# scalar-labs/jepsen

Hardware: AMD Instinct MI355X
Metric: history ops verified/sec (node), independent cas-register 10k keys, 1/2/4/8 GPU (higher is better)
Workload: dtype int64

## Files before the change

jepsen_amd/csrc/jh_lin.hip:

```cpp
#include "jh_internal.h"
#include <hipcub/hipcub.hpp>
#include <algorithm>
#include <type_traits>
#include "lin/lin_common.h"

namespace {

constexpr int F_READ = 0, F_WRITE = 1, F_CAS = 2, F_OTHER = 4;
constexpr int T_INVOKE = 0, T_OK = 1, T_FAIL = 2, T_INFO = 3;
constexpr uint64_t VIOL_NONE = ~0ULL;
#ifndef JH_LDS_TBL
#define JH_LDS_TBL 0
#endif
constexpr int LDS_TBL = JH_LDS_TBL;
#ifdef JH_STEP_PROF
#define PROF_MARK(v) const unsigned long long v = __builtin_amdgcn_s_memtime()
#define PROF_ADD(acc, a, b) acc += (b) - (a)
#else
#define PROF_MARK(v)
#define PROF_ADD(acc, a, b)
#endif
#ifdef JH_DFS_STATS
#define DFS_STAT(x) x
#else
#define DFS_STAT(x)
#endif
template <int LG_BKT, int LG_BLOOM>
struct MemoCfg {
    static constexpr int LG = LG_BKT;
    static constexpr int BKT = 1 << LG_BKT;
    static constexpr int SLOTS = BKT * 4;
    static constexpr int EVICT = SLOTS * 5 / 8;
    static constexpr int BLOOM = 1 << LG_BLOOM;
    static constexpr int OFF_MEMO = LDS_TBL;
    static constexpr int OFF_BLOOM = OFF_MEMO + SLOTS * 8;
    static constexpr int OFF_CNT = OFF_BLOOM + BLOOM / 8;
    static constexpr int LDS = OFF_CNT + BKT;
};
#ifndef JH_MEMOQ_LG
#define JH_MEMOQ_LG 7
#define JH_MEMOQ_BLOOM 14
#endif
using MemoQ = MemoCfg<JH_MEMOQ_LG, JH_MEMOQ_BLOOM>;
#ifndef JH_MEMOH_BLOOM
#define JH_MEMOH_BLOOM 17
#endif
using MemoH = MemoCfg<12, JH_MEMOH_BLOOM>;
using MemoM = MemoCfg<10, 15>;
#ifndef JH_P2_LG
#define JH_P2_LG 10
#define JH_P2_BLOOM 17
#endif
#ifndef JH_P2_PER_CU
#define JH_P2_PER_CU 3
#endif
using MemoP2 = MemoCfg<JH_P2_LG, JH_P2_BLOOM>;
constexpr int P2_DENSE_PER_CU = 6;
using MemoP2D = MemoCfg<9, 16>;
constexpr int P2_LEAN_PER_CU = P2_DENSE_PER_CU;
constexpr int STATE_BITS = 20, T_BITS = 20, GEN_BITS = 24;
constexpr uint32_t STATE_MASK = (1u << STATE_BITS) - 1, T_MASK = (1u << T_BITS) - 1;

struct Rec {
    int32_t proc;
    uint8_t type, f;
    uint16_t pad;
    int32_t v1, v2;
};

struct Op {
    int32_t v1, v2;
    int32_t rr;
    int32_t fa;
// ... 641 lines not shown
#endif
__device__ __forceinline__ uint32_t hbm_insert(uint64_t *memo, uint32_t cap_mask, uint32_t gen,
                                               uint32_t ct, uint32_t cs, uint64_t cm) {
    uint32_t b = (uint32_t)memo_hash(ct, cs, cm) & cap_mask & ~(HB - 1);
    const uint64_t w1 = ((uint64_t)gen << 40) | ((uint64_t)ct << 20) | cs;
    for (;;) {
        const ulonglong2 *B = (const ulonglong2 *)(memo + 2 * (size_t)b);
        ulonglong2 e[HB];
#pragma unroll
        for (uint32_t j = 0; j < HB; j++) e[j] = B[j];
        int j0 = -1;
        unsigned long long exp = 0;
#pragma unroll
        for (int j = HB - 1; j >= 0; j--)
            if ((e[j].y >> 40) != gen) { j0 = j; exp = e[j].y; }
        if (j0 < 0) { b = (b + HB) & cap_mask; continue; }
        if (__hip_atomic_compare_exchange_strong((unsigned long long *)&memo[2 * (size_t)(b + j0) + 1],
                                                 &exp, (unsigned long long)w1,
                                                 __ATOMIC_RELAXED, __ATOMIC_RELAXED,
                                                 __HIP_MEMORY_SCOPE_WORKGROUP)) {
            __hip_atomic_store(&memo[2 * (size_t)(b + j0)], cm, __ATOMIC_RELAXED,
                               __HIP_MEMORY_SCOPE_WORKGROUP);
#ifdef JH_DUP_WRITE
            if (g_dup_base)
                g_dup_base[((uintptr_t)&memo[2 * (size_t)(b + j0)] >> 4) & ((1u << 26) - 1)] = make_ulonglong2(cm, w1);
#endif
            return b + (uint32_t)j0;
        }
    }
}

__device__ __forceinline__ uint64_t hbm_probe(const uint64_t *memo, uint32_t cap_mask, uint32_t gen,
                                              uint32_t ct, uint32_t cs, uint64_t cm,
                                              unsigned long long &probes) {
    const uint64_t w1want = ((uint64_t)gen << 40) | ((uint64_t)ct << 20) | cs;
    uint32_t b = (uint32_t)memo_hash(ct, cs, cm) & cap_mask & ~(HB - 1);
    for (;;) {
        const ulonglong2 *B = (const ulonglong2 *)(memo + 2 * (size_t)b);
        ulonglong2 e[HB];
#pragma unroll
        for (uint32_t j = 0; j < HB; j++) e[j] = B[j];
        probes++;
        int empty = -1, hit = -1;
#pragma unroll
        for (int j = HB - 1; j >= 0; j--) {
            if ((e[j].y >> 40) != gen) empty = j;
            if (e[j].y == w1want && e[j].x == cm) hit = j;
        }
        if (hit >= 0 && (empty < 0 || hit < empty)) return b + (uint32_t)hit;
        if (empty >= 0) return (1ULL << 32) | (b + (uint32_t)empty);
        b = (b + HB) & cap_mask;
    }
}

__device__ __forceinline__ uint32_t lk_t(uint64_t k) { return (uint32_t)(k >> 48) & 0x3FFF; }
__device__ __forceinline__ uint32_t lk_s(uint64_t k) { return (uint32_t)(k >> 40) & 0xFF; }
__device__ __forceinline__ uint64_t lk_m(uint64_t k) { return k & ((1ULL << 40) - 1); }
__device__ __forceinline__ void lk_hash(uint32_t klo, uint32_t khi, uint32_t &h1, uint32_t &h2) {
    h1 = (klo ^ __builtin_rotateleft32(khi, 16)) * 0x9E3779B1u;
    h2 = (klo + __builtin_rotateleft32(khi, 5)) * 0x85EBCA77u;
}
template <class M>
__device__ __forceinline__ void lk_bkts(uint32_t h1, uint32_t h2, uint32_t &b1, uint32_t &b2) {
    b1 = h1 >> (32 - M::LG);
    b2 = h2 >> (32 - M::LG);
}
__device__ __forceinline__ uint32_t lk_bl(uint32_t h) { return h ^ (h >> 15); }

template <class M>
__device__ __noinline__ uint64_t memo_evict(uint64_t *lmemo, uint32_t *bcnt, uint32_t *bloom,
                                            uint64_t *memo, uint64_t *stage,
                                            uint32_t cap_mask, uint32_t gen, uint32_t t_cur,
                                            uint32_t theta_old, int lane,
                                            uint32_t *hlog = nullptr, uint32_t hlog_cap = 0, uint32_t nlog = 0) {
    static_assert(M::SLOTS < 65536, "kept fits 16 bits");
    int bins = 0;
#pragma unroll 1
    for (int r = 0; r < M::SLOTS / 64; r++) {
        const uint64_t x = lmemo[lane + 64 * r];
        stage[lane + 64 * r] = x;
        const uint32_t xt = lk_t(x);
        const int d = x == 0 ? 99 : (xt >= t_cur ? 0 : (int)min(t_cur - xt, 15u));
#pragma unroll
        for (int b = 0; b < 16; b++) {
            const int cnt = __popcll(ballot(d == b));
            if (lane == b) bins += cnt;
        }
    }
    int acc = 0, dstar = -1;
#pragma unroll 1
    for (int b = 0; b < 16; b++) {
        acc += readlane(bins, b);
        if (acc > M::EVICT / 2) break;
        dstar = b;
    }
    uint32_t th2;
    if (dstar < 0) th2 = t_cur + 1;
    else {
        th2 = t_cur > (uint32_t)dstar ? t_cur - (uint32_t)dstar : 0u;
        if (dstar == 15) th2 = t_cur - min(t_cur, 15u);
    }
    th2 = max(th2, theta_old);
    wave_sync();
#pragma unroll 1
    for (int r = 0; r < M::SLOTS / 64; r++) lmemo[lane + 64 * r] = 0;
    for (int i = lane; i < M::BKT / 4; i += 64) bcnt[i] = 0;
// ... 330 lines not shown
                    const uint32_t x = (uint32_t)readlane((int)drq, (int)(u - 1 - tb0));
                    if (lane == ru) wrq = x;
                    w++;
                }
                t = pt;
                r = lay_hi(t) & 63;
                DFS_STAT(n_reload++);
            }
            PROF_MARK(q5); PROF_ADD(pc_pop, q2, q5);
        }
        if (depth >= A.stack_cap) { verdict = JH_UNKNOWN; if (lane == 0) atomicOr(A.flags, QF_STACK_OVERFLOW); break; }
    }
    inserts = ins;
    tmax_out = tmax;
#ifdef JH_STEP_PROF
    if (A.dbg && lane == 0) {
        unsigned long long *d = A.dbg + 16 * (size_t)blockIdx.x;
        d[10] += pc_lift; d[11] += pc_probe; d[12] += pc_ins; d[13] += pc_fwd; d[14] += pc_pop;
        d[0] += pc_cand; d[1] += pc_key; d[8] += pc_lds;
    }
#endif
#ifdef JH_DFS_STATS
    if (A.dbg && lane == 0) {
        unsigned long long *d = A.dbg + 16 * (size_t)blockIdx.x;
        d[4] += n_steps; d[5] += (unsigned long long)ins; d[6] += n_evict; d[7] += n_reload; d[9] += n_slow;
    }
#endif
    return verdict;
}

template <class M, bool HO = false>
__device__ __forceinline__ int dfs_lean(const DfsArgs &A, const KeyInfo &K, const char *tb, int key, int lane,
                        uint64_t *memo, Frame *stack, uint64_t *stage,
                        long long &inserts, uint32_t &tmax_out, unsigned long long &my_probes,
                        uint32_t &ins_real, uint32_t *hlog) {
    const OpC *ops = (const OpC *)tb;
    const Lay *lay = (const Lay *)(tb + tblc_ops_bytes(K));
    const uint32_t n_ok = (uint32_t)K.n_ok;
    const int n_ops = K.n_ops;
    const uint32_t cap_mask = A.memo_cap - 1;
    const uint32_t gen = (A.gen_base + (uint32_t)key + 1) & ((1u << GEN_BITS) - 1);
    uint64_t *lmemo = (uint64_t *)(jh_lds + M::OFF_MEMO);
    uint32_t *bloom = (uint32_t *)(jh_lds + M::OFF_BLOOM);
    uint32_t *bcnt = (uint32_t *)(jh_lds + M::OFF_CNT);
    uint8_t *bcnt8 = (uint8_t *)bcnt;
    for (int i = lane; i < M::SLOTS; i += 64) lmemo[i] = 0;
    for (int i = lane; i < M::BKT / 4; i += 64) bcnt[i] = 0;
    for (int i = lane; i < M::BLOOM / 32; i += 64) bloom[i] = 0;
    const uint32_t lb_lo = lane < 32 ? 1u << lane : 0u, lb_hi = lane >= 32 ? 1u << (lane - 32) : 0u;
    uint32_t theta = 0;
    int lcount = 0;
    uint32_t n_steps = 0, n_lay = 0, n_up = 0, n_spill = 0, n_refill = 0, n_slow = 0, n_evict = 0, n_hbm = 0;
    const unsigned long long probes0 = my_probes;

    uint32_t tb0 = 0, drq = 0, dhi = 0;
    auto load_lay = [&](uint32_t base) {
        DFS_STAT(n_lay++);
        tb0 = base;
        const uint32_t u = base + (uint32_t)lane;
        if (u < n_ok) { const Lay e = lay[u]; drq = e.rq; dhi = e.hi; }
    };
    auto lay_hi = [&](uint32_t u) -> uint32_t {
        if (u - tb0 >= 64u) load_lay(u >= 32 ? u - 32 : 0);
        return (uint32_t)readlane((int)dhi, (int)(u - tb0));
    };
    int pb = 0;
    uint32_t urq = RQ_EMPTY;
    auto load_up = [&](int base) {
        DFS_STAT(n_up++);
        pb = base;
        const int j = base + lane;
        urq = j < n_ops ? ops[j].rq : RQ_EMPTY;
    };
    uint32_t fm_lo = 0, fm_hi = 0, f_ti = 0, f_s = 0, fr_lo = 0, fr_hi = 0;

    load_lay(0);
    uint32_t t = 0, tmax = 0, depth = 0, ring_lo = 0;
    uint64_t mask = 0;
    uint32_t s = (uint32_t)A.init_state;
    int verdict = -1;
    uint32_t ins = 0;
    uint32_t budget = (uint32_t)min<int64_t>(A.budget, 0x7FFFFFFF);
    uint32_t chk = min(budget, 1023u);
    int w = (int)(lay_hi(0) >> 6), P = w;
    uint32_t r = lay_hi(0) & 63;
    uint32_t rn = n_ok > 1 ? (lay_hi(1) & 63) : 0;
    uint32_t wrq = lane < w ? ops[lane].rq : RQ_EMPTY;
    load_up(P);
    wave_sync();
    uint32_t ins_saved = 0xFFFFFFFFu;
    uint32_t nlog = 0;
    uint32_t stall_base = 0, stall_tmax = 0;
    bool ho = false;
    unsigned long long ho_off = 0;
    auto advance = [&](uint32_t nt) {
        for (uint32_t u = t; u < nt; u++) {
            const uint32_t ru = u == t ? r : (lay_hi(u) & 63);
            const uint32_t sh = (uint32_t)wave_shl1((int)wrq);
            if (lane >= (int)ru) wrq = sh;
            w--;
            if (lane == w) wrq = RQ_EMPTY;
            const int c = (int)(lay_hi(u + 1) >> 6);
            if (c > 0) {
                if (P < pb || P + c > pb + 64) load_up(c <= 32 && P >= 32 ? P - 32 : P);
                for (int kk = 0; kk < c; kk++) {
                    const uint32_t x = (uint32_t)readlane((int)urq, P - pb + kk);
                    if (lane == w + kk) wrq = x;
                }
                w += c; P += c;
            }
        }
    };
    if (A.rs_mode == 2 && A.rs_off) {
        const int64_t ro = A.rs_off[key];
        if (ro >= 0) {
            const uint64_t *hd = (const uint64_t *)(A.rs_arena + ro);
            const uint64_t h_mask = hd[0], h_ts = hd[1], h_dt = hd[2], h_ins = hd[3], h_n = hd[4];
            const uint32_t d = (uint32_t)h_dt;
            if (d <= A.stack_cap && h_n <= (uint64_t)A.memo_cap / 4) {
                const Frame *fsrc = (const Frame *)(hd + 8);
                const ulonglong2 *ent = (const ulonglong2 *)(fsrc + d);
                uint32_t tmx = 0;
                for (uint32_t j = (uint32_t)lane; j < (uint32_t)h_n; j += 64) {
                    const ulonglong2 e = ent[j];
                    const uint32_t et = (uint32_t)(e.y >> 20) & T_MASK, es = (uint32_t)e.y & STATE_MASK;
                    const uint32_t sl = hbm_insert(memo, cap_mask, gen, et, es, e.x);
                    if constexpr (HO) { if (hlog && j < A.hlog_cap) hlog[j] = sl; } else (void)sl;
                    uint32_t g1, g2;
                    lk_hash((uint32_t)e.x, (uint32_t)(e.x >> 32) | (et << 16) | (es << 8) | 0x80000000u, g1, g2);
                    bloom_set2<M>(bloom, lk_bl(g1), lk_bl(g2));
                    tmx = max(tmx, et + 1);
                }
                for (int o = 32; o > 0; o >>= 1) tmx = max(tmx, (uint32_t)__shfl_xor((int)tmx, o));
                theta = rflu(tmx);
                if constexpr (HO) nlog = (uint32_t)min<uint64_t>(h_n, 0xFFFFu);
                ring_lo = d > 32 ? d - 32 : 0;
                for (uint32_t j = (uint32_t)lane; j < ring_lo; j += 64) stack[j] = fsrc[j];
                {
                    const uint32_t idx = ring_lo + (((uint32_t)lane - ring_lo) & 63);
                    if (idx < d) {
                        const Frame fr = fsrc[idx];
                        fm_lo = (uint32_t)fr.mask; fm_hi = (uint32_t)(fr.mask >> 32); f_ti = fr.t_i;
                        f_s = (uint32_t)fr.s; fr_lo = (uint32_t)fr.rest; fr_hi = (uint32_t)(fr.rest >> 32);
                    }
                }
                __builtin_amdgcn_fence(__ATOMIC_RELEASE, "workgroup");
                __builtin_amdgcn_fence(__ATOMIC_ACQUIRE, "workgroup");
                wave_sync();
                depth = d;
                mask = h_mask;
                s = (uint32_t)(h_ts >> 32);
                ins = (uint32_t)h_ins;
                chk = min(budget, ins);
                const uint32_t nt = (uint32_t)h_ts;
                advance(nt);
                t = nt;
                tmax = max((uint32_t)(h_dt >> 32), t);
                r = lay_hi(t) & 63;
                rn = t + 1 < n_ok ? (lay_hi(t + 1) & 63) : 0;
                stall_base = ins; stall_tmax = tmax;
            }
        }
    }
    const ulonglong2 *B = (const ulonglong2 *)lmemo;
    uint64_t absent = 0, nm_r = 0;
    uint32_t u_r = 0, klo = 0, khi = 0, b1 = 0, b2 = 0, n1 = 0, n2 = 0, h1 = 0, h2 = 0, nvl = 0;
    auto child_keys = [&]() {
        u_r = t; nm_r = 0;
        if ((absent >> r) & 1) {
            uint64_t nm = drop_bit(mask, r);
            uint32_t u = t + 1;
            if (u >= n_ok) nm = 0;
            else if ((nm >> rn) & 1) {
                uint32_t ru = rn;
                for (;;) {
                    nm = drop_bit(nm, ru);
                    u++;
                    if (u >= n_ok) { nm = 0; break; }
                    ru = lay_hi(u) & 63;
                    if (!((nm >> ru) & 1)) break;
                }
            }
            u_r = u; nm_r = nm;
        }
        nvl = wrq >> 16;
        const bool is_r = lane == (int)r;
        const uint32_t hi_a = (uint32_t)(mask >> 32) | (t << 16) | 0x80000000u;
        const uint32_t hi_r = (uint32_t)(nm_r >> 32) | (u_r << 16) | 0x80000000u;
        klo = is_r ? (uint32_t)nm_r : ((uint32_t)mask | lb_lo);
        khi = (is_r ? hi_r : (hi_a | lb_hi)) | (nvl << 8);
        lk_hash(klo, khi, h1, h2);
        lk_bkts<M>(h1, h2, b1, b2);
    };

expand:
    DFS_STAT(n_steps++);
    {
        const uint32_t req = wrq & 0xFFFF;
        absent = (ballot(req == s) | ballot(req == RQ_ANY)) & ~mask;
    }
    if (!absent) goto pop;
    child_keys();
    {
        const bool cl = (absent >> lane) & 1;
        const uint32_t a1 = cl ? b1 : 0u, a2 = cl ? b2 : 0u;
        const uint64_t k = ((uint64_t)khi << 32) | klo;
        n1 = bcnt8[a1]; n2 = bcnt8[a2];
        __builtin_amdgcn_sched_barrier(0);
        const ulonglong2 x0 = B[2 * a1], x1 = B[2 * a1 + 1];
        const ulonglong2 y0 = B[2 * a2], y1 = B[2 * a2 + 1];
        const uint64_t hit = ballot(x0.x == k) | ballot(x0.y == k) | ballot(x1.x == k) | ballot(x1.y == k) |
                             ballot(y0.x == k) | ballot(y0.y == k) | ballot(y1.x == k) | ballot(y1.y == k);
        absent &= ~hit;
        if (t < theta && absent) {
            DFS_STAT(n_slow++);
            uint64_t low = absent;
            if (u_r >= theta) low &= ~(1ULL << r);
            const uint32_t kt = khi >> 16 & 0x7FFF, ks = (khi >> 8) & 0xFF;
            const uint64_t km = k & ((1ULL << 40) - 1);
            const bool maybe = ((low >> lane) & 1) && bloom_test2<M>(bloom, lk_bl(h1), lk_bl(h2));
            bool found = false;
            if (maybe) found = (hbm_probe(memo, cap_mask, gen, kt, ks, km, my_probes) >> 32) == 0;
            absent &= ~ballot(found);
        }
    }
    if (!absent) goto pop;

insert:
    {
        if (ins >= chk) {
            if (ins >= budget && !extend_budget(A, budget)) { verdict = JH_UNKNOWN; goto done; }
            if (handover(A, ins)) { ins_saved = ins; ins = budget; verdict = JH_UNKNOWN; goto done; }
            if (A.claim) {
                int c = 0;
                if (lane == 0) c = __hip_atomic_load(&A.claim[key], __ATOMIC_RELAXED, __HIP_MEMORY_SCOPE_AGENT);
                if (readlane(c, 0)) { verdict = JH_CANCELLED; goto done; }
            }
            if (A.prio_ins > 0 && ins >= (uint32_t)A.prio_ins) {
                if (ins >= 4u * (uint32_t)A.prio_ins) __builtin_amdgcn_s_setprio(3);
                else if (ins >= 2u * (uint32_t)A.prio_ins) __builtin_amdgcn_s_setprio(2);
                else __builtin_amdgcn_s_setprio(1);
            }
            if (!std::is_same<M, MemoQ>::value && A.stall) {
                if (tmax > stall_tmax) { stall_tmax = tmax; stall_base = ins; }
                if (lane == 0)
                    __hip_atomic_store(&A.stall[key], ins - stall_base, __ATOMIC_RELAXED, __HIP_MEMORY_SCOPE_AGENT);
            }
            if (HO && A.handoff) {
                int h = 0;
                if (lane == 0) h = __hip_atomic_load(&A.handoff[key], __ATOMIC_RELAXED, __HIP_MEMORY_SCOPE_AGENT);
                if (readlane(h, 0) == HO_ASK) {
                    bool ok = hlog && nlog <= A.hlog_cap && ins <= A.memo_cap / 4;
                    if (ok) {
                        const uint64_t bytes = 64 + (uint64_t)depth * sizeof(Frame) + (uint64_t)ins * 16;
                        unsigned long long off = 0;
                        if (lane == 0) off = atomicAdd(A.rs_used, (unsigned long long)((bytes + 255) & ~255ULL));
                        ho_off = readlane64(off, 0);
                        ok = ho_off + bytes <= A.rs_cap;
                    }
                    int won = 0;
                    if (lane == 0) {
                        int exp = HO_ASK;
                        won = __hip_atomic_compare_exchange_strong(&A.handoff[key], &exp, ok ? HO_SAVING : HO_REFUSED,
                                                                   __ATOMIC_RELAXED, __ATOMIC_RELAXED,
                                                                   __HIP_MEMORY_SCOPE_AGENT) ? 1 : 0;
                    }
                    if (readlane(won, 0) && ok) { ho = true; goto done; }
                }
            }
            chk = min(budget, ins + (HO && A.handoff ? 256u : 1024u));
        }
        const int i = __builtin_ctzll(absent);
        ins++;
        const uint32_t ns = (uint32_t)readlane((int)nvl, i);
        const bool to_r = (uint32_t)i == r;
        const uint32_t nt = to_r ? u_r : t;
        {
            const bool pick1 = n1 <= n2;
            const uint32_t bs = pick1 ? b1 : b2, nsl = pick1 ? n1 : n2;
            const uint64_t full_m = ballot(nsl >= 4);
            if (!((full_m >> i) & 1)) {
                if (lane == i) {
                    lmemo[4 * bs + nsl] = ((uint64_t)khi << 32) | klo;
                    bcnt8[bs] = (uint8_t)(nsl + 1);
                }
                if (++lcount >= M::EVICT) {
                    DFS_STAT(n_evict++);
                    const uint64_t er = memo_evict<M>(lmemo, bcnt, bloom, memo, stage, cap_mask, gen, nt, theta, lane,
                                                      hlog, A.hlog_cap, nlog);
                    DFS_STAT(n_hbm += (uint32_t)lcount - ((uint32_t)er & 0xFFFF));
                    lcount = rfl((int)((uint32_t)er & 0xFFFF));
                    nlog = rflu(((uint32_t)er >> 16) & 0xFFFF);
                    theta = rflu((uint32_t)(er >> 32));
                }
            } else {
                const uint64_t nmask = to_r ? nm_r : (mask | (1ULL << i));
                if (lane == i) {
                    const uint32_t sl = hbm_insert(memo, cap_mask, gen, nt, ns, nmask);
                    bloom_set2<M>(bloom, lk_bl(h1), lk_bl(h2));
                    if (hlog && nlog < A.hlog_cap) hlog[nlog] = sl;
                }
                nlog = min(nlog + 1, 0xFFFFu);
                __builtin_amdgcn_fence(__ATOMIC_RELEASE, "workgroup");
                __builtin_amdgcn_fence(__ATOMIC_ACQUIRE, "workgroup");
                theta = max(theta, nt + 1);
                DFS_STAT(n_hbm++);
            }
        }
        if (depth - ring_lo == 64) {
            DFS_STAT(n_spill++);
            const uint32_t kk = ((uint32_t)lane - ring_lo) & 63;
            if (kk < 32) {
                Frame fr;
                fr.mask = ((uint64_t)fm_hi << 32) | fm_lo; fr.t_i = f_ti; fr.s = (int32_t)f_s;
                fr.rest = ((uint64_t)fr_hi << 32) | fr_lo; fr.pad[0] = fr.pad[1] = 0;
                stack[ring_lo + kk] = fr;
            }
            ring_lo += 32;
        }
        {
            const uint64_t nrest = absent & (absent - 1);
            const bool me = lane == (int)(depth & 63);
            fm_lo = me ? (uint32_t)mask : fm_lo;
            fm_hi = me ? (uint32_t)(mask >> 32) : fm_hi;
            f_ti = me ? ((t << 6) | (uint32_t)i) : f_ti;
            f_s = me ? s : f_s;
            fr_lo = me ? (uint32_t)nrest : fr_lo;
            fr_hi = me ? (uint32_t)(nrest >> 32) : fr_hi;
        }
        depth++;
        s = ns;
        if (!to_r) {
            mask |= 1ULL << i;
            goto expand;
        }
        mask = nm_r;
        if (nt >= n_ok) { t = nt; tmax = max(tmax, t); verdict = JH_VALID; goto done; }
        advance(nt);
        t = nt;
        if (t > tmax) {
            tmax = t;
            if (A.stamp_progress && A.seq_start && lane == 0)
                __hip_atomic_store(&A.seq_start[key], __builtin_amdgcn_s_memrealtime() | 1ULL, __ATOMIC_RELAXED,
                                   __HIP_MEMORY_SCOPE_AGENT);
        }
        r = lay_hi(t) & 63;
        rn = t + 1 < n_ok ? (lay_hi(t + 1) & 63) : 0;
        goto expand;
    }

pop:
    DFS_STAT(n_steps++);
    if (depth == ring_lo) {
        if (depth == 0) { verdict = JH_INVALID; goto done; }
        DFS_STAT(n_refill++);
        __builtin_amdgcn_fence(__ATOMIC_RELEASE, "workgroup");
        __builtin_amdgcn_fence(__ATOMIC_ACQUIRE, "workgroup");
        const uint32_t lo = depth >= 32 ? depth - 32 : 0;
        const uint32_t kk = ((uint32_t)lane - lo) & 63;
        if (kk < depth - lo) {
            const Frame fr = stack[lo + kk];
            fm_lo = (uint32_t)fr.mask; fm_hi = (uint32_t)(fr.mask >> 32); f_ti = fr.t_i; f_s = (uint32_t)fr.s;
            fr_lo = (uint32_t)fr.rest; fr_hi = (uint32_t)(fr.rest >> 32);
        }
        ring_lo = lo;
    }
    depth--;
    {
        const int ln = (int)(depth & 63);
        absent = ((uint64_t)(uint32_t)readlane((int)fr_hi, ln) << 32) | (uint32_t)readlane((int)fr_lo, ln);
        const uint32_t pt = (uint32_t)readlane((int)f_ti, ln) >> 6;
        mask = ((uint64_t)(uint32_t)readlane((int)fm_hi, ln) << 32) | (uint32_t)readlane((int)fm_lo, ln);
        s = (uint32_t)readlane((int)f_s, ln);
        if (pt != t) {
            for (uint32_t u = t; u > pt; u--) {
                const int c = (int)(lay_hi(u) >> 6);
                w -= c; P -= c;
                if (lane >= w) wrq = RQ_EMPTY;
                const uint32_t h = lay_hi(u - 1);
                const int ru = (int)(h & 63);
                const uint32_t sh = (uint32_t)wave_shr1((int)wrq);
                if (lane > ru) wrq = sh;
                const uint32_t x = (uint32_t)readlane((int)drq, (int)(u - 1 - tb0));
                if (lane == ru) wrq = x;
                w++;
            }
            t = pt;
            r = lay_hi(t) & 63;
            rn = t + 1 < n_ok ? (lay_hi(t + 1) & 63) : 0;
        }
    }
    if (!absent) goto pop;
    child_keys();
    {
        const bool cl = (absent >> lane) & 1;
        const uint32_t a1 = cl ? b1 : 0u, a2 = cl ? b2 : 0u;
        n1 = bcnt8[a1]; n2 = bcnt8[a2];
    }
    goto insert;

done:
    if ((A.rs_mode == 1 && A.rs_off && verdict == JH_UNKNOWN && A.defer) || (HO && ho)) {
        const uint32_t nmem = ins_saved != 0xFFFFFFFFu ? ins_saved : ins;
        const uint64_t bytes = 64 + (uint64_t)depth * sizeof(Frame) + (uint64_t)nmem * 16;
        unsigned long long off = 0;
        if (HO && ho) off = ho_off;
        else {
            if (lane == 0) off = atomicAdd(A.rs_used, (unsigned long long)((bytes + 255) & ~255ULL));
            off = readlane64(off, 0);
        }
        if (off + bytes <= A.rs_cap) {
            uint64_t *hd = (uint64_t *)(A.rs_arena + off);
            Frame *fdst = (Frame *)(hd + 8);
            ulonglong2 *ent = (ulonglong2 *)(fdst + depth);
            for (uint32_t j = (uint32_t)lane; j < ring_lo; j += 64) fdst[j] = stack[j];
            {
                const uint32_t idx = ring_lo + (((uint32_t)lane - ring_lo) & 63);
                if (idx < depth) {
                    Frame fr;
                    fr.mask = ((uint64_t)fm_hi << 32) | fm_lo; fr.t_i = f_ti; fr.s = (int32_t)f_s;
                    fr.rest = ((uint64_t)fr_hi << 32) | fr_lo; fr.pad[0] = fr.pad[1] = 0;
                    fdst[idx] = fr;
                }
            }
            __builtin_amdgcn_fence(__ATOMIC_RELEASE, "workgroup");
            __builtin_amdgcn_fence(__ATOMIC_ACQUIRE, "workgroup");
            uint32_t n = 0;
            for (int base = 0; base < M::SLOTS; base += 64) {
                const uint64_t x = lmemo[base + lane];
                const uint64_t bm = ballot(x != 0);
                const uint32_t at = n + (uint32_t)mbcnt(bm);
                if (x != 0 && at < nmem) ent[at] = make_ulonglong2(lk_m(x), ((uint64_t)lk_t(x) << 20) | lk_s(x));
                n += (uint32_t)__popcll(bm);
            }
            const ulonglong2 *tab = (const ulonglong2 *)memo;
            if (hlog && nlog <= A.hlog_cap) {
                for (uint32_t base = 0; base < nlog; base += 64 * 8) {
                    ulonglong2 e[8];
#pragma unroll
                    for (int q = 0; q < 8; q++) {
                        const uint32_t j = base + 64 * q + (uint32_t)lane;
                        e[q] = j < nlog ? tab[hlog[j]] : make_ulonglong2(0ULL, 0ULL);
                    }
#pragma unroll
                    for (int q = 0; q < 8; q++) {
                        const bool mine = base + 64 * q + (uint32_t)lane < nlog && (uint32_t)(e[q].y >> 40) == gen;
                        const uint64_t bm = ballot(mine);
                        const uint32_t at = n + (uint32_t)mbcnt(bm);
                        if (mine && at < nmem) ent[at] = make_ulonglong2(e[q].x, e[q].y & ((1ULL << 40) - 1));
                        n += (uint32_t)__popcll(bm);
                    }
                }
            } else
            for (uint32_t base = 0; base < A.memo_cap; base += 64 * 16) {
                ulonglong2 e[16];
#pragma unroll
                for (int q = 0; q < 16; q++) e[q] = tab[base + 64 * q + lane];
#pragma unroll
                for (int q = 0; q < 16; q++) {
                    const bool mine = (uint32_t)(e[q].y >> 40) == gen;
                    const uint64_t bm = ballot(mine);
                    const uint32_t at = n + (uint32_t)mbcnt(bm);
                    if (mine && at < nmem) ent[at] = make_ulonglong2(e[q].x, e[q].y & ((1ULL << 40) - 1));
                    n += (uint32_t)__popcll(bm);
                }
            }
            if (lane == 0) {
                hd[0] = mask; hd[1] = (uint64_t)t | ((uint64_t)s << 32); hd[2] = (uint64_t)depth | ((uint64_t)tmax << 32);
                hd[3] = nmem; hd[4] = n;
            }
            __builtin_amdgcn_fence(__ATOMIC_RELEASE, "agent");
            if (lane == 0 && n == nmem) {
                A.rs_off[key] = (int64_t)off;
                atomicAdd((int32_t *)A.rs_used + ((ho ? Q_RS_TAKEOVERS : Q_RS_PUBLISHED) - Q_RS_USED), 1);
            }
            if (ho && lane == 0) {
                __builtin_amdgcn_fence(__ATOMIC_RELEASE, "agent");
                __hip_atomic_store(&A.handoff[key], n == nmem ? HO_DONE : HO_REFUSED, __ATOMIC_RELEASE,
                                   __HIP_MEMORY_SCOPE_AGENT);
            }
            if (HO && ho && n != nmem) { ins = 0; verdict = JH_CANCELLED; ho = false; }
        } else if (ho) {
            if (lane == 0) __hip_atomic_store(&A.handoff[key], HO_REFUSED, __ATOMIC_RELEASE, __HIP_MEMORY_SCOPE_AGENT);
            verdict = JH_CANCELLED; ho = false;
        }
    }
    if (HO && ho) return V_HANDED;
    inserts = ins;
    ins_real = ins_saved != 0xFFFFFFFFu ? ins_saved : ins;
    tmax_out = tmax;
#ifdef JH_DFS_STATS
    if (A.dbg && lane == 0) {
        unsigned long long *d = A.dbg + 16 * (size_t)blockIdx.x;
        d[4] += n_steps; d[5] += ins; d[6] += n_evict; d[7] += n_lay; d[10] += n_up;
        d[11] += n_spill; d[12] += n_refill; d[13] += n_slow; d[14] += my_probes - probes0; d[8] += n_hbm;
    }
#endif
    return verdict;
}

__device__ __forceinline__ uint32_t w_t(uint64_t y) { return (uint32_t)(y >> 16) & 0x7FFF; }
__device__ __forceinline__ uint32_t w_s(uint64_t y) { return (uint32_t)y & 0xFFFF; }
__device__ __forceinline__ void w_hash(uint64_t m, uint32_t y, uint32_t &h1, uint32_t &h2) {
    const uint32_t lo = (uint32_t)m, hi = (uint32_t)(m >> 32);
    h1 = (lo ^ __builtin_rotateleft32(hi, 16) ^ __builtin_rotateleft32(y, 8)) * 0x9E3779B1u;
    h2 = (lo + __builtin_rotateleft32(hi, 5) + __builtin_rotateleft32(y, 11)) * 0x85EBCA77u;
}

template <class M>
__device__ __noinline__ uint64_t memo_evict_w(ulonglong2 *lmemo, uint32_t *bcnt, uint32_t *bloom, uint64_t *memo,
                                              ulonglong2 *stage, uint32_t cap_mask, uint32_t gen, uint32_t t_cur,
                                              uint32_t theta_old, int lane) {
    int bins = 0;
#pragma unroll 1
    for (int r = 0; r < M::SLOTS / 64; r++) {
        const ulonglong2 x = lmemo[lane + 64 * r];
        stage[lane + 64 * r] = x;
        const uint32_t xt = w_t(x.y);
        const int d = x.y == 0 ? 99 : (xt >= t_cur ? 0 : (int)min(t_cur - xt, 15u));
#pragma unroll
        for (int b = 0; b < 16; b++) {
            const int cnt = __popcll(ballot(d == b));
            if (lane == b) bins += cnt;
        }
    }
    int acc = 0, dstar = -1;
#pragma unroll 1
    for (int b = 0; b < 16; b++) {
        acc += readlane(bins, b);
        if (acc > M::EVICT / 2) break;
        dstar = b;
    }
    uint32_t th2;
    if (dstar < 0) th2 = t_cur + 1;
    else {
        th2 = t_cur > (uint32_t)dstar ? t_cur - (uint32_t)dstar : 0u;
        if (dstar == 15) th2 = t_cur - min(t_cur, 15u);
    }
    th2 = max(th2, theta_old);
    wave_sync();
#pragma unroll 1
    for (int r = 0; r < M::SLOTS / 64; r++) lmemo[lane + 64 * r] = make_ulonglong2(0, 0);
    for (int i = lane; i < M::BKT / 4; i += 64) bcnt[i] = 0;
// ... 5275 lines not shown
```

jepsen_amd/csrc/lin/lin_diag.h:

```cpp
#pragma once

namespace {

void LinRun::diag_phase1_waves() {
    if (!dbg2) return;
    std::vector<unsigned long long> h((size_t)waves1 * 16);
    HIP_TRY(hipMemcpy(h.data(), dbg, h.size() * 8, hipMemcpyDeviceToHost));
    unsigned long long tot[16] = {0}, mx9 = 0;
    for (int w = 0; w < waves1; w++) { for (int k = 0; k < 16; k++) tot[k] += h[16 * w + k]; mx9 = std::max(mx9, h[16 * w + 9]); }
    fprintf(stderr, "[jh-dfs] waves=%d keys=%llu search=%.0f cyc/key | steps=%llu inserts=%llu evict=%llu lay-loads=%llu op-loads=%llu spills=%llu refills=%llu slow=%llu hbm-probes=%llu hbm-inserts=%llu | cyc/step=%.0f | wave-busy avg=%.0f max=%llu cyc\n",
            waves1, tot[3], (double)tot[2] / std::max(1ULL, tot[3]), tot[4], tot[5], tot[6], tot[7], tot[10],
            tot[11], tot[12], tot[13], tot[14], tot[8], (double)tot[2] / std::max(1ULL, tot[4]), (double)tot[9] / waves1, mx9);
    HIP_TRY(hipMemsetAsync(dbg, 0, sizeof(unsigned long long) * (waves1 + 512) * 16, st));
}

void LinRun::diag_helper_keys() {
    if (!(n_help > 0 && wh.key_prof)) return;
    HIP_TRY(hipStreamSynchronize(st));
    std::vector<unsigned long long> kp(3 * (size_t)K);
    HIP_TRY(hipMemcpy(kp.data(), wh.key_prof, kp.size() * 8, hipMemcpyDeviceToHost));
    for (int64_t k = 0; k < K; k++)
        if (kp[3 * k])
            fprintf(stderr, "[jh-help] key %lld wg %llu verdict %llu won %llu inserts %llu cycles %llu end_us %llu\n",
                    (long long)k, (kp[3 * k + 2] >> 8) & 0xFFF, kp[3 * k + 2] & 0xFF, (kp[3 * k + 2] >> 20) & 1,
                    kp[3 * k + 1], kp[3 * k], kp[3 * k + 2] >> 32);
}

void LinRun::diag_bfs_dump() {
    const char *dp = tune_env("JH_BFS_DUMP");
    if (!dp) return;
    HIP_TRY(hipStreamSynchronize(st));
    std::vector<uint64_t> nd(c.ncap);
    HIP_TRY(hipMemcpy(nd.data(), c.nodes, nd.size() * 8, hipMemcpyDeviceToHost));
    if (FILE *fp = fopen(dp, "wb")) { fwrite(nd.data(), 8, nd.size(), fp); fclose(fp); }
}

void LinRun::diag_race_waves() {
    if (!dbg2) return;
    HIP_TRY(hipMemcpyAsync(qh, q, sizeof qh, hipMemcpyDeviceToHost, st));
    HIP_TRY(hipStreamSynchronize(st));
    n_unres = qh[Q_UNRES];
    std::vector<unsigned long long> h((size_t)wg2 * 16);
    HIP_TRY(hipMemcpy(h.data(), dbg, h.size() * 8, hipMemcpyDeviceToHost));
    for (int w = 0; w < wg2; w++)
        if (h[16 * w + 4])
            fprintf(stderr, "[jh-bfs] wg %d keys=%llu cycles=%llu rounds=%llu configs=%llu cyc/round=%.0f | "
                    "count: hash=%llu live=%llu path=%llu closure=%llu cyc | global-set rounds=%llu cyc=%llu "
                    "configs=%llu, LDS-set rounds cyc=%llu configs=%llu | live: layers=%llu (LDS %llu) head-cyc=%llu LDS-layers-cyc=%llu\n",
                    w, h[16 * w + 4], h[16 * w], h[16 * w + 1], h[16 * w + 3],
                    (double)h[16 * w] / std::max(1ULL, h[16 * w + 1]), h[16 * w + 5], h[16 * w + 6],
                    h[16 * w + 7], h[16 * w + 8], h[16 * w + 10], h[16 * w + 9], h[16 * w + 11],
                    h[16 * w + 12], h[16 * w + 13], h[16 * w + 14] & 0xFFFFFFFF, h[16 * w + 14] >> 32, h[16 * w + 15], h[16 * w + 2]);
#ifdef JH_BFS_PROF
    {
        unsigned long long bp[8];
        HIP_TRY(hipMemcpyFromSymbol(bp, HIP_SYMBOL(g_bfs_prof), sizeof bp));
        const double nr = (double)std::max(1ULL, bp[4]), nl = (double)std::max(1ULL, bp[6]);
        unsigned long long bx[4];
        HIP_TRY(hipMemcpyFromSymbol(bx, HIP_SYMBOL(g_bfs_prof_x), sizeof bx));
        const double ni = (double)std::max(1ULL, bx[2]);
        fprintf(stderr, "[jh-bfs-prof] rounds=%llu cyc/round: claim+barrier %.0f items %.0f barrier %.0f tail %.0f | "
                "layers=%llu formation cyc/layer %.0f | tid0 items=%llu cyc/item: load+children %.0f insert8 %.0f record8 %.0f\n",
                bp[4], bp[0] / nr, bp[1] / nr, bp[2] / nr, bp[3] / nr, bp[6], bp[5] / nl, bx[2], bp[7] / ni, bx[0] / ni, bx[1] / ni);
        memset(bx, 0, sizeof bx);
        HIP_TRY(hipMemcpyToSymbol(HIP_SYMBOL(g_bfs_prof_x), bx, sizeof bx));
        memset(bp, 0, sizeof bp);
        HIP_TRY(hipMemcpyToSymbol(HIP_SYMBOL(g_bfs_prof), bp, sizeof bp));
    }
#endif
    std::vector<unsigned long long> g((size_t)waves2 * 16);
    HIP_TRY(hipMemcpy(g.data(), dbg + 16 * 256, g.size() * 8, hipMemcpyDeviceToHost));
    for (int w = 0; w < waves2; w++)
        if (g[16 * w + 4] > 0)
            fprintf(stderr, "[jh-seq] wave %d keys=%llu search=%llu cyc busy=%llu | steps=%llu inserts=%llu evict=%llu lay-loads=%llu op-loads=%llu spills=%llu refills=%llu slow=%llu hbm-probes=%llu | cyc/step=%.0f\n",
                    w, g[16 * w + 3], g[16 * w + 2], g[16 * w + 9], g[16 * w + 4], g[16 * w + 5], g[16 * w + 6],
                    g[16 * w + 7], g[16 * w + 10], g[16 * w + 11], g[16 * w + 12], g[16 * w + 13], g[16 * w + 14],
                    (double)g[16 * w + 2] / std::max(1ULL, g[16 * w + 4]));
}

void LinRun::diag_defer_timeline() {
    if (!(defer_times && n_defer > 0)) return;
    HIP_TRY(hipStreamSynchronize(st));
    if (stream_p2) {
        int32_t nd = 0;
        HIP_TRY(hipMemcpy(&nd, q + Q_DEFER, sizeof nd, hipMemcpyDeviceToHost));
        n_defer = nd;
    }
    std::vector<unsigned long long> dt((size_t)K + 2);
    HIP_TRY(hipMemcpy(dt.data(), a.defer_time, dt.size() * 8, hipMemcpyDeviceToHost));
    std::vector<int32_t> dk(n_defer);
    HIP_TRY(hipMemcpy(dk.data(), defer, sizeof(int32_t) * n_defer, hipMemcpyDeviceToHost));
    std::vector<jh_key_verdict> vv(K);
    HIP_TRY(hipMemcpy(vv.data(), out_dev, sizeof(jh_key_verdict) * K, hipMemcpyDeviceToHost));
    std::vector<unsigned long long> ss;
    if (ctx->bufs.size() > WS_HELP_START && ctx->bufs[WS_HELP_START].p) {
        ss.resize(K);
        HIP_TRY(hipMemcpy(ss.data(), ctx->bufs[WS_HELP_START].p, 8 * K, hipMemcpyDeviceToHost));
    }
    fprintf(stderr, "[jh-defer] phase 1: %.1f us (first wave start to last wave end)\n", (dt[1] - dt[0]) / 100.0);
    std::vector<std::pair<double, int>> ev;
    for (int d = 0; d < n_defer; d++) ev.push_back({(dt[2 + dk[d]] - dt[0]) / 100.0, dk[d]});
    std::vector<std::pair<long long, int>> heavy;
    for (int d = 0; d < n_defer; d++) heavy.push_back({vv[dk[d]].explored, dk[d]});
    std::sort(heavy.rbegin(), heavy.rend());
    std::vector<unsigned long long> tl;
    if (ctx->bufs.size() > WS_TL && ctx->bufs[WS_TL].p) {
        tl.resize(TL_W * (size_t)K);
        HIP_TRY(hipMemcpy(tl.data(), ctx->bufs[WS_TL].p, 8 * tl.size(), hipMemcpyDeviceToHost));
    }
    auto us = [&](unsigned long long t) { return t ? (double)(t - dt[0]) / 100.0 : -1.0; };
    for (int i = 0; i < std::min(n_defer, 12); i++) {
        const int k = heavy[i].second;
        double st_us = -1;
        if (!ss.empty() && ss[k] && ss[k] != SEQ_HANDED) st_us = ((ss[k] & ~1ULL) - dt[0]) / 100.0;
        fprintf(stderr, "[jh-defer] key %d explored %lld valid %d deferred %.1f us seq-start %.1f us", k,
                heavy[i].first, vv[k].valid, (dt[2 + k] - dt[0]) / 100.0, st_us);
        if (!tl.empty())
            fprintf(stderr, " | bfs %.1f-%.1f us seq %.1f-%.1f us", us(tl[TL_W * k]), us(tl[TL_W * k + 1]),
                    us(tl[TL_W * k + 2]), us(tl[TL_W * k + 3]));
        fprintf(stderr, "\n");
    }
    if (!tl.empty()) {
        std::vector<std::pair<unsigned long long, int>> last;
        for (int d = 0; d < n_defer; d++) {
// ... 149 lines not shown
```

Baseline: 259.9 million.

## Fuse bloom/HBM probe issue with LDS lookup, push frame first, split step profiling

For the non-MemoQ memo config, the kernel now reads the bloom words and issues the HBM memo probe loads alongside the LDS bucket reads. This overlaps global-memory latency with the LDS hit check instead of probing only after a miss. It also pushes the parent frame before the memo insert, makes budget and header values scalar via readfirstlane, replaces repeated lay_hi window checks with a single cover check per step, and makes the stack refill branchless. An optional lean per-phase cycle profiler is added; in exchange, speculative HBM loads are issued even for children that later hit in LDS.

Result: no change. 261.6 million (median of 6 runs) (+0.7%).

```diff
diff --git a/jepsen_amd/csrc/jh_lin.hip b/jepsen_amd/csrc/jh_lin.hip
--- a/jepsen_amd/csrc/jh_lin.hip
+++ b/jepsen_amd/csrc/jh_lin.hip
@@ -19,6 +19,17 @@
 #else
 #define PROF_MARK(v)
 #define PROF_ADD(acc, a, b)
+#endif
+#if defined(JH_STEP_PROF) && !defined(JH_DFS_STATS)
+#define JH_LEAN_SPLIT 1
+#define LEAN_LAP(acc) do { \
+        __builtin_amdgcn_sched_barrier(0); \
+        const unsigned long long lp_n = __builtin_amdgcn_s_memtime(); \
+        lp.acc += lp_n - lp.t; lp.t = lp_n; \
+        __builtin_amdgcn_sched_barrier(0); \
+    } while (0)
+#else
+#define LEAN_LAP(acc) do { } while (0)
 #endif
 #ifdef JH_DFS_STATS
 #define DFS_STAT(x) x
@@ -766,6 +777,34 @@
         b = (b + HB) & cap_mask;
     }
 }
+__device__ __forceinline__ uint32_t hbm_probe_issue(const uint64_t *memo, uint32_t cap_mask, uint32_t ct, uint32_t cs,
+                                                    uint64_t cm, ulonglong2 (&e)[HB]) {
+    const uint32_t b = (uint32_t)memo_hash(ct, cs, cm) & cap_mask & ~(HB - 1);
+    const ulonglong2 *B = (const ulonglong2 *)(memo + 2 * (size_t)b);
+#pragma unroll
+    for (uint32_t j = 0; j < HB; j++) e[j] = B[j];
+    return b;
+}
+__device__ __forceinline__ uint64_t hbm_probe_take(const uint64_t *memo, uint32_t cap_mask, uint32_t gen,
+                                                   uint32_t ct, uint32_t cs, uint64_t cm, uint32_t b,
+                                                   ulonglong2 (&e)[HB], unsigned long long &probes) {
+    const uint64_t w1want = ((uint64_t)gen << 40) | ((uint64_t)ct << 20) | cs;
+    for (;;) {
+        probes++;
+        int empty = -1, hit = -1;
+#pragma unroll
+        for (int j = HB - 1; j >= 0; j--) {
+            if ((e[j].y >> 40) != gen) empty = j;
+            if (e[j].y == w1want && e[j].x == cm) hit = j;
+        }
+        if (hit >= 0 && (empty < 0 || hit < empty)) return b + (uint32_t)hit;
+        if (empty >= 0) return (1ULL << 32) | (b + (uint32_t)empty);
+        b = (b + HB) & cap_mask;
+        const ulonglong2 *B = (const ulonglong2 *)(memo + 2 * (size_t)b);
+#pragma unroll
+        for (uint32_t j = 0; j < HB; j++) e[j] = B[j];
+    }
+}
 
 __device__ __forceinline__ uint32_t lk_t(uint64_t k) { return (uint32_t)(k >> 48) & 0x3FFF; }
 __device__ __forceinline__ uint32_t lk_s(uint64_t k) { return (uint32_t)(k >> 40) & 0xFF; }
@@ -1202,6 +1241,11 @@
     int lcount = 0;
     uint32_t n_steps = 0, n_lay = 0, n_up = 0, n_spill = 0, n_refill = 0, n_slow = 0, n_evict = 0, n_hbm = 0;
     const unsigned long long probes0 = my_probes;
+    constexpr bool FUSED_SLOW = !std::is_same<M, MemoQ>::value;
+    constexpr bool PUSH_FIRST = !std::is_same<M, MemoQ>::value;
+#ifdef JH_LEAN_SPLIT
+    struct { unsigned long long t, head, lds, hit, bloom, hbm, ins, adv, popf, popb, popc; uint32_t steps, ins0; } lp = {};
+#endif
 
     uint32_t tb0 = 0, drq = 0, dhi = 0;
     auto load_lay = [&](uint32_t base) {
@@ -1231,7 +1275,9 @@
     int verdict = -1;
     uint32_t ins = 0;
     uint32_t budget = (uint32_t)min<int64_t>(A.budget, 0x7FFFFFFF);
+    if constexpr (!std::is_same<M, MemoQ>::value) budget = rflu(budget);
     uint32_t chk = min(budget, 1023u);
+    if constexpr (!std::is_same<M, MemoQ>::value) chk = rflu(chk);
     int w = (int)(lay_hi(0) >> 6), P = w;
     uint32_t r = lay_hi(0) & 63;
     uint32_t rn = n_ok > 1 ? (lay_hi(1) & 63) : 0;
@@ -1243,14 +1289,19 @@
     uint32_t stall_base = 0, stall_tmax = 0;
     bool ho = false;
     unsigned long long ho_off = 0;
+    auto lay_cover3 = [&](uint32_t lo) {
+        if (lo - tb0 >= 62u) load_lay(lo >= 31 ? lo - 31 : 0);
+    };
+    auto lay_at = [&](uint32_t u) -> uint32_t { return (uint32_t)readlane((int)dhi, (int)(u - tb0)); };
     auto advance = [&](uint32_t nt) {
         for (uint32_t u = t; u < nt; u++) {
-            const uint32_t ru = u == t ? r : (lay_hi(u) & 63);
+            lay_cover3(u);
+            const uint32_t ru = u == t ? r : (lay_at(u) & 63);
             const uint32_t sh = (uint32_t)wave_shl1((int)wrq);
             if (lane >= (int)ru) wrq = sh;
             w--;
             if (lane == w) wrq = RQ_EMPTY;
-            const int c = (int)(lay_hi(u + 1) >> 6);
+            const int c = (int)(lay_at(u + 1) >> 6);
             if (c > 0) {
                 if (P < pb || P + c > pb + 64) load_up(c <= 32 && P >= 32 ? P - 32 : P);
                 for (int kk = 0; kk < c; kk++) {
@@ -1265,7 +1316,8 @@
         const int64_t ro = A.rs_off[key];
         if (ro >= 0) {
             const uint64_t *hd = (const uint64_t *)(A.rs_arena + ro);
-            const uint64_t h_mask = hd[0], h_ts = hd[1], h_dt = hd[2], h_ins = hd[3], h_n = hd[4];
+            const uint64_t h_mask = rfl64(hd[0]), h_ts = rfl64(hd[1]), h_dt = rfl64(hd[2]), h_ins = rfl64(hd[3]),
+                           h_n = rfl64(hd[4]);
             const uint32_t d = (uint32_t)h_dt;
             if (d <= A.stack_cap && h_n <= (uint64_t)A.memo_cap / 4) {
                 const Frame *fsrc = (const Frame *)(hd + 8);
@@ -1343,35 +1395,80 @@
         lk_bkts<M>(h1, h2, b1, b2);
     };
 
+#ifdef JH_LEAN_SPLIT
+    lp.ins0 = ins;
+    lp.t = __builtin_amdgcn_s_memtime();
+#endif
+
 expand:
     DFS_STAT(n_steps++);
+#ifdef JH_LEAN_SPLIT
+    lp.steps++;
+#endif
     {
         const uint32_t req = wrq & 0xFFFF;
         absent = (ballot(req == s) | ballot(req == RQ_ANY)) & ~mask;
     }
-    if (!absent) goto pop;
+    if (!absent) { LEAN_LAP(head); goto pop; }
     child_keys();
-    {
+    if (FUSED_SLOW && t < theta) {
         const bool cl = (absent >> lane) & 1;
         const uint32_t a1 = cl ? b1 : 0u, a2 = cl ? b2 : 0u;
         const uint64_t k = ((uint64_t)khi << 32) | klo;
+        const uint32_t p1 = lk_bl(h1) & (M::BLOOM - 1), p2 = lk_bl(h2) & (M::BLOOM - 1);
+        LEAN_LAP(head);
+        const uint32_t w1 = bloom[p1 >> 5], w2 = bloom[p2 >> 5];
         n1 = bcnt8[a1]; n2 = bcnt8[a2];
         __builtin_amdgcn_sched_barrier(0);
         const ulonglong2 x0 = B[2 * a1], x1 = B[2 * a1 + 1];
         const ulonglong2 y0 = B[2 * a2], y1 = B[2 * a2 + 1];
+        __builtin_amdgcn_sched_barrier(0);
+        DFS_STAT(n_slow++);
+        uint64_t low = absent;
+        if (u_r >= theta) low &= ~(1ULL << r);
+        const uint32_t kt = khi >> 16 & 0x7FFF, ks = (khi >> 8) & 0xFF;
+        const uint64_t km = k & ((1ULL << 40) - 1);
+        const bool maybe = ((low >> lane) & 1) && ((w1 >> (p1 & 31)) & (w2 >> (p2 & 31)) & 1u) != 0;
+        ulonglong2 e[HB];
+        uint32_t hb = 0;
+        if (maybe) hb = hbm_probe_issue(memo, cap_mask, kt, ks, km, e);
+        __builtin_amdgcn_sched_barrier(0);
+        LEAN_LAP(bloom);
         const uint64_t hit = ballot(x0.x == k) | ballot(x0.y == k) | ballot(x1.x == k) | ballot(x1.y == k) |
                              ballot(y0.x == k) | ballot(y0.y == k) | ballot(y1.x == k) | ballot(y1.y == k);
         absent &= ~hit;
-        if (t < theta && absent) {
+        LEAN_LAP(hit);
+        bool found = false;
+        if (maybe && ((absent >> lane) & 1))
+            found = (hbm_probe_take(memo, cap_mask, gen, kt, ks, km, hb, e, my_probes) >> 32) == 0;
+        absent &= ~ballot(found);
+        LEAN_LAP(hbm);
+    } else {
+        const bool cl = (absent >> lane) & 1;
+        const uint32_t a1 = cl ? b1 : 0u, a2 = cl ? b2 : 0u;
+        const uint64_t k = ((uint64_t)khi << 32) | klo;
+        LEAN_LAP(head);
+        n1 = bcnt8[a1]; n2 = bcnt8[a2];
+        __builtin_amdgcn_sched_barrier(0);
+        const ulonglong2 x0 = B[2 * a1], x1 = B[2 * a1 + 1];
+        const ulonglong2 y0 = B[2 * a2], y1 = B[2 * a2 + 1];
+        LEAN_LAP(lds);
+        const uint64_t hit = ballot(x0.x == k) | ballot(x0.y == k) | ballot(x1.x == k) | ballot(x1.y == k) |
+                             ballot(y0.x == k) | ballot(y0.y == k) | ballot(y1.x == k) | ballot(y1.y == k);
+        absent &= ~hit;
+        LEAN_LAP(hit);
+        if (!FUSED_SLOW && t < theta && absent) {
             DFS_STAT(n_slow++);
             uint64_t low = absent;
             if (u_r >= theta) low &= ~(1ULL << r);
             const uint32_t kt = khi >> 16 & 0x7FFF, ks = (khi >> 8) & 0xFF;
             const uint64_t km = k & ((1ULL << 40) - 1);
             const bool maybe = ((low >> lane) & 1) && bloom_test2<M>(bloom, lk_bl(h1), lk_bl(h2));
+            LEAN_LAP(bloom);
             bool found = false;
             if (maybe) found = (hbm_probe(memo, cap_mask, gen, kt, ks, km, my_probes) >> 32) == 0;
             absent &= ~ballot(found);
+            LEAN_LAP(hbm);
         }
     }
     if (!absent) goto pop;
@@ -1425,38 +1522,7 @@
         const uint32_t ns = (uint32_t)readlane((int)nvl, i);
         const bool to_r = (uint32_t)i == r;
         const uint32_t nt = to_r ? u_r : t;
-        {
-            const bool pick1 = n1 <= n2;
-            const uint32_t bs = pick1 ? b1 : b2, nsl = pick1 ? n1 : n2;
-            const uint64_t full_m = ballot(nsl >= 4);
-            if (!((full_m >> i) & 1)) {
-                if (lane == i) {
-                    lmemo[4 * bs + nsl] = ((uint64_t)khi << 32) | klo;
-                    bcnt8[bs] = (uint8_t)(nsl + 1);
-                }
-                if (++lcount >= M::EVICT) {
-                    DFS_STAT(n_evict++);
-                    const uint64_t er = memo_evict<M>(lmemo, bcnt, bloom, memo, stage, cap_mask, gen, nt, theta, lane,
-                                                      hlog, A.hlog_cap, nlog);
-                    DFS_STAT(n_hbm += (uint32_t)lcount - ((uint32_t)er & 0xFFFF));
-                    lcount = rfl((int)((uint32_t)er & 0xFFFF));
-                    nlog = rflu(((uint32_t)er >> 16) & 0xFFFF);
-                    theta = rflu((uint32_t)(er >> 32));
-                }
-            } else {
-                const uint64_t nmask = to_r ? nm_r : (mask | (1ULL << i));
-                if (lane == i) {
-                    const uint32_t sl = hbm_insert(memo, cap_mask, gen, nt, ns, nmask);
-                    bloom_set2<M>(bloom, lk_bl(h1), lk_bl(h2));
-                    if (hlog && nlog < A.hlog_cap) hlog[nlog] = sl;
-                }
-                nlog = min(nlog + 1, 0xFFFFu);
-                __builtin_amdgcn_fence(__ATOMIC_RELEASE, "workgroup");
-                __builtin_amdgcn_fence(__ATOMIC_ACQUIRE, "workgroup");
-                theta = max(theta, nt + 1);
-                DFS_STAT(n_hbm++);
-            }
-        }
+        auto push_parent = [&]() {
         if (depth - ring_lo == 64) {
             DFS_STAT(n_spill++);
             const uint32_t kk = ((uint32_t)lane - ring_lo) & 63;
@@ -1479,7 +1545,43 @@
             fr_hi = me ? (uint32_t)(nrest >> 32) : fr_hi;
         }
         depth++;
+        };
+        if constexpr (PUSH_FIRST) push_parent();
+        {
+            const bool pick1 = n1 <= n2;
+            const uint32_t bs = pick1 ? b1 : b2, nsl = pick1 ? n1 : n2;
+            const uint64_t full_m = ballot(nsl >= 4);
+            if (!((full_m >> i) & 1)) {
+                if (lane == i) {
+                    lmemo[4 * bs + nsl] = ((uint64_t)khi << 32) | klo;
+                    bcnt8[bs] = (uint8_t)(nsl + 1);
+                }
+                if (++lcount >= M::EVICT) {
+                    DFS_STAT(n_evict++);
+                    const uint64_t er = memo_evict<M>(lmemo, bcnt, bloom, memo, stage, cap_mask, gen, nt, theta, lane,
+                                                      hlog, A.hlog_cap, nlog);
+                    DFS_STAT(n_hbm += (uint32_t)lcount - ((uint32_t)er & 0xFFFF));
+                    lcount = rfl((int)((uint32_t)er & 0xFFFF));
+                    nlog = rflu(((uint32_t)er >> 16) & 0xFFFF);
+                    theta = rflu((uint32_t)(er >> 32));
+                }
+            } else {
+                const uint64_t nmask = to_r ? nm_r : (mask | (1ULL << i));
+                if (lane == i) {
+                    const uint32_t sl = hbm_insert(memo, cap_mask, gen, nt, ns, nmask);
+                    bloom_set2<M>(bloom, lk_bl(h1), lk_bl(h2));
+                    if (hlog && nlog < A.hlog_cap) hlog[nlog] = sl;
+                }
+                nlog = min(nlog + 1, 0xFFFFu);
+                __builtin_amdgcn_fence(__ATOMIC_RELEASE, "workgroup");
+                __builtin_amdgcn_fence(__ATOMIC_ACQUIRE, "workgroup");
+                theta = max(theta, nt + 1);
+                DFS_STAT(n_hbm++);
+            }
+        }
+        if constexpr (!PUSH_FIRST) push_parent();
         s = ns;
+        LEAN_LAP(ins);
         if (!to_r) {
             mask |= 1ULL << i;
             goto expand;
@@ -1494,13 +1596,17 @@
                 __hip_atomic_store(&A.seq_start[key], __builtin_amdgcn_s_memrealtime() | 1ULL, __ATOMIC_RELAXED,
                                    __HIP_MEMORY_SCOPE_AGENT);
         }
-        r = lay_hi(t) & 63;
-        rn = t + 1 < n_ok ? (lay_hi(t + 1) & 63) : 0;
+        r = lay_at(t) & 63;
+        rn = t + 1 < n_ok ? (lay_at(t + 1) & 63) : 0;
+        LEAN_LAP(adv);
         goto expand;
     }
 
 pop:
     DFS_STAT(n_steps++);
+#ifdef JH_LEAN_SPLIT
+    lp.steps++;
+#endif
     if (depth == ring_lo) {
         if (depth == 0) { verdict = JH_INVALID; goto done; }
         DFS_STAT(n_refill++);
@@ -1508,11 +1614,11 @@
         __builtin_amdgcn_fence(__ATOMIC_ACQUIRE, "workgroup");
         const uint32_t lo = depth >= 32 ? depth - 32 : 0;
         const uint32_t kk = ((uint32_t)lane - lo) & 63;
-        if (kk < depth - lo) {
-            const Frame fr = stack[lo + kk];
-            fm_lo = (uint32_t)fr.mask; fm_hi = (uint32_t)(fr.mask >> 32); f_ti = fr.t_i; f_s = (uint32_t)fr.s;
-            fr_lo = (uint32_t)fr.rest; fr_hi = (uint32_t)(fr.rest >> 32);
-        }
+        const bool in = kk < depth - lo;
+        const Frame fr = stack[in ? lo + kk : depth - 1];
+        fm_lo = in ? (uint32_t)fr.mask : fm_lo; fm_hi = in ? (uint32_t)(fr.mask >> 32) : fm_hi;
+        f_ti = in ? fr.t_i : f_ti; f_s = in ? (uint32_t)fr.s : f_s;
+        fr_lo = in ? (uint32_t)fr.rest : fr_lo; fr_hi = in ? (uint32_t)(fr.rest >> 32) : fr_hi;
         ring_lo = lo;
     }
     depth--;
@@ -1522,12 +1628,15 @@
         const uint32_t pt = (uint32_t)readlane((int)f_ti, ln) >> 6;
         mask = ((uint64_t)(uint32_t)readlane((int)fm_hi, ln) << 32) | (uint32_t)readlane((int)fm_lo, ln);
         s = (uint32_t)readlane((int)f_s, ln);
+        LEAN_LAP(popf);
         if (pt != t) {
+            uint32_t h = 0;
             for (uint32_t u = t; u > pt; u--) {
-                const int c = (int)(lay_hi(u) >> 6);
+                lay_cover3(u - 1);
+                const int c = (int)(lay_at(u) >> 6);
                 w -= c; P -= c;
                 if (lane >= w) wrq = RQ_EMPTY;
-                const uint32_t h = lay_hi(u - 1);
+                h = lay_at(u - 1);
                 const int ru = (int)(h & 63);
                 const uint32_t sh = (uint32_t)wave_shr1((int)wrq);
                 if (lane > ru) wrq = sh;
@@ -1536,9 +1645,10 @@
                 w++;
             }
             t = pt;
-            r = lay_hi(t) & 63;
-            rn = t + 1 < n_ok ? (lay_hi(t + 1) & 63) : 0;
-        }
+            r = h & 63;
+            rn = t + 1 < n_ok ? (lay_at(t + 1) & 63) : 0;
+        }
+        LEAN_LAP(popb);
     }
     if (!absent) goto pop;
     child_keys();
@@ -1547,6 +1657,7 @@
         const uint32_t a1 = cl ? b1 : 0u, a2 = cl ? b2 : 0u;
         n1 = bcnt8[a1]; n2 = bcnt8[a2];
     }
+    LEAN_LAP(popc);
     goto insert;
 
 done:
@@ -1639,6 +1750,14 @@
     inserts = ins;
     ins_real = ins_saved != 0xFFFFFFFFu ? ins_saved : ins;
     tmax_out = tmax;
+#ifdef JH_LEAN_SPLIT
+    if (A.dbg && lane == 0) {
+        unsigned long long *d = A.dbg + 16 * (size_t)blockIdx.x;
+        d[4] += lp.steps; d[5] += (ins_saved != 0xFFFFFFFFu ? ins_saved : ins) - lp.ins0;
+        d[0] += lp.head; d[1] += lp.lds; d[6] += lp.hit; d[7] += lp.bloom; d[8] += lp.hbm;
+        d[10] += lp.ins; d[11] += lp.adv; d[12] += lp.popf; d[13] += lp.popb; d[14] += lp.popc;
+    }
+#endif
 #ifdef JH_DFS_STATS
     if (A.dbg && lane == 0) {
         unsigned long long *d = A.dbg + 16 * (size_t)blockIdx.x;
diff --git a/jepsen_amd/csrc/lin/lin_diag.h b/jepsen_amd/csrc/lin/lin_diag.h
--- a/jepsen_amd/csrc/lin/lin_diag.h
+++ b/jepsen_amd/csrc/lin/lin_diag.h
@@ -1,6 +1,18 @@
 #pragma once
 
 namespace {
+
+#ifdef JH_LEAN_SPLIT
+static void diag_lean_split(const char *tag, int w, const unsigned long long *g) {
+    const double st = (double)std::max(1ULL, g[4]);
+    const unsigned long long sum = g[0] + g[1] + g[6] + g[7] + g[8] + g[10] + g[11] + g[12] + g[13] + g[14];
+    fprintf(stderr, "[%s-split] wave %d steps=%llu inserts=%llu steps/insert=%.2f cyc/step=%.0f | cyc/step: head+keys %.0f "
+            "lds-wait %.0f hit %.0f bloom %.0f hbm %.0f insert+push %.0f advance %.0f pop-frame %.0f pop-window %.0f "
+            "pop-fill %.0f\n",
+            tag, w, g[4], g[5], (double)g[4] / (double)std::max(1ULL, g[5]), sum / st, g[0] / st, g[1] / st, g[6] / st,
+            g[7] / st, g[8] / st, g[10] / st, g[11] / st, g[12] / st, g[13] / st, g[14] / st);
+}
+#endif
 
 void LinRun::diag_phase1_waves() {
     if (!dbg2) return;
@@ -8,6 +20,11 @@
     HIP_TRY(hipMemcpy(h.data(), dbg, h.size() * 8, hipMemcpyDeviceToHost));
     unsigned long long tot[16] = {0}, mx9 = 0;
     for (int w = 0; w < waves1; w++) { for (int k = 0; k < 16; k++) tot[k] += h[16 * w + k]; mx9 = std::max(mx9, h[16 * w + 9]); }
+#ifdef JH_LEAN_SPLIT
+    diag_lean_split("jh-dfs", waves1, tot);
+    HIP_TRY(hipMemsetAsync(dbg, 0, sizeof(unsigned long long) * (waves1 + 512) * 16, st));
+    return;
+#endif
     fprintf(stderr, "[jh-dfs] waves=%d keys=%llu search=%.0f cyc/key | steps=%llu inserts=%llu evict=%llu lay-loads=%llu op-loads=%llu spills=%llu refills=%llu slow=%llu hbm-probes=%llu hbm-inserts=%llu | cyc/step=%.0f | wave-busy avg=%.0f max=%llu cyc\n",
             waves1, tot[3], (double)tot[2] / std::max(1ULL, tot[3]), tot[4], tot[5], tot[6], tot[7], tot[10],
             tot[11], tot[12], tot[13], tot[14], tot[8], (double)tot[2] / std::max(1ULL, tot[4]), (double)tot[9] / waves1, mx9);
@@ -70,6 +87,15 @@
 #endif
     std::vector<unsigned long long> g((size_t)waves2 * 16);
     HIP_TRY(hipMemcpy(g.data(), dbg + 16 * 256, g.size() * 8, hipMemcpyDeviceToHost));
+#ifdef JH_LEAN_SPLIT
+    for (int w = 0; w < waves2; w++)
+        if (g[16 * w + 4] > 0) {
+            fprintf(stderr, "[jh-seq] wave %d keys=%llu search=%llu cyc busy=%llu\n", w, g[16 * w + 3], g[16 * w + 2],
+                    g[16 * w + 9]);
+            diag_lean_split("jh-seq", w, &g[16 * (size_t)w]);
+        }
+    return;
+#endif
     for (int w = 0; w < waves2; w++)
         if (g[16 * w + 4] > 0)
             fprintf(stderr, "[jh-seq] wave %d keys=%llu search=%llu cyc busy=%llu | steps=%llu inserts=%llu evict=%llu lay-loads=%llu op-loads=%llu spills=%llu refills=%llu slow=%llu hbm-probes=%llu | cyc/step=%.0f\n",
```
